# PhilippKath/concentus

Measured on NVIDIA B200. Metric: CELT decode audio-sec per sec (x realtime), 48k stereo, higher is better.
Workload: dtype int32

## Files before the change

concentus_b200/csrc/celt_bands.cuh:

```cuda
#pragma once
#include "celt_pvq.cuh"
#include "celt_rate.cuh"

namespace cb {

struct BandCtx {
    EcDec ec;
    int16_t *tmp;
    int i;
    int intensity, spread, tf_change;
    int remaining_bits;
    unsigned seed;
    bool dry;
};

struct SplitCtx {
    int inv, imid, iside, delta, itheta, qalloc;
};


CB_DEV_NOINLINE void haar1(int16_t *X, int N0, int stride) {
    N0 >>= 1;
    CB_NOUNROLL for (int i = 0; i < stride; i++)
        CB_NOUNROLL for (int j = 0; j < N0; j++) {
            int a = stride * 2 * j + i, b = stride * (2 * j + 1) + i;
            int t1 = mul16_16(23170, X[a]);
            int t2 = mul16_16(23170, X[b]);
            X[a] = (int16_t)pshr32(wadd(t1, t2), 15);
            X[b] = (int16_t)pshr32(wsub(t1, t2), 15);
        }
}

CB_DEV_NOINLINE void deinterleave_hadamard(int16_t *__restrict__ X, int16_t *__restrict__ tmp, int N0, int stride, int hadamard) {
    const int N = N0 * stride;
    const uint8_t *ordery = kOrdery + stride - 2;
    CB_NOUNROLL for (int i = 0; i < stride; i++) {
        const int row = hadamard ? ordery[i] : i;
        int16_t *d = tmp + row * N0;
        const int16_t *x = X + i;
        CB_NOUNROLL for (int j = 0; j < N0; j++) d[j] = x[j * stride];
    }
    CB_NOUNROLL for (int p = 0; p < N; p++) X[p] = tmp[p];
}
CB_DEV_NOINLINE void interleave_hadamard(int16_t *__restrict__ X, int16_t *__restrict__ tmp, int N0, int stride, int hadamard) {
    const int N = N0 * stride;
    const uint8_t *ordery = kOrdery + stride - 2;
    CB_NOUNROLL for (int i = 0; i < stride; i++) {
        const int row = hadamard ? ordery[i] : i;
        int16_t *d = tmp + i;
        const int16_t *x = X + row * N0;
        CB_NOUNROLL for (int j = 0; j < N0; j++) d[j * stride] = x[j];
    }
    CB_NOUNROLL for (int p = 0; p < N; p++) X[p] = tmp[p];
}

CB_DEV_NOINLINE void stereo_merge(int16_t *__restrict__ X, int16_t *__restrict__ Y, int mid, int N) {
    int xp = 0, side = 0;
    CB_NOUNROLL for (int j = 0; j < N; j++) {
        xp = mac16_16(xp, Y[j], X[j]);
        side = mac16_16(side, Y[j], Y[j]);
    }
    xp = mul16_32_q15(mid, xp);
    int mid2 = s16(mid >> 1);
    int El = wsub(wadd(mul16_16(mid2, mid2), side), wmul(2, xp));
    int Er = wadd(wadd(mul16_16(mid2, mid2), side), wmul(2, xp));
    if (Er < 161061 || El < 161061) {
        CB_NOUNROLL for (int j = 0; j < N; j++) Y[j] = X[j];
        return;
    }
    int kl = celt_ilog2(El) >> 1;
    int kr = celt_ilog2(Er) >> 1;
    int t = vshr32(El, (kl - 7) << 1);
    int lgain = celt_rsqrt_norm(t);
    t = vshr32(Er, (kr - 7) << 1);
    int rgain = celt_rsqrt_norm(t);
    if (kl < 7) kl = 7;
    if (kr < 7) kr = 7;
    CB_NOUNROLL for (int j = 0; j < N; j++) {
        int l = s16(mul16_16_p15(mid, X[j]));
        int r = Y[j];
        X[j] = (int16_t)pshr32(mul16_16(lgain, s16(l - r)), kl + 1);
        Y[j] = (int16_t)pshr32(mul16_16(rgain, s16(l + r)), kr + 1);
    }
}

CB_DEV int compute_qn(int N, int b, int offset, int pulse_cap, int stereo) {
    int N2 = 2 * N - 1;
    if (stereo && N == 2) N2--;
    int qb = sudiv(b + N2 * offset, N2);
    qb = imin(b - pulse_cap - (4 << kBitRes), qb);
    qb = imin(8 << kBitRes, qb);
    int qn;
    if (qb < (1 << kBitRes >> 1)) {
        qn = 1;
    } else {
        qn = kExp2Table8[qb & 0x7] >> (14 - (qb >> kBitRes));
        qn = (qn + 1) >> 1 << 1;
    }
    return qn;
}

CB_DEV void compute_theta(BandCtx &ctx, SplitCtx &sctx, int N, int *b, int B, int B0, int LM, int stereo, int *fill) {
    EcDec &ec = ctx.ec;
    int itheta = 0, inv = 0;
    int pulse_cap = kLogN[ctx.i] + LM * (1 << kBitRes);
    int offset = (pulse_cap >> 1) - (stereo && N == 2 ? kQThetaOffsetTwoPhase : kQThetaOffset);
    int qn = compute_qn(N, *b, offset, pulse_cap, stereo);
    if (stereo && ctx.i >= ctx.intensity) qn = 1;
    int tell = (int)ec.tell_frac();
    if (qn != 1) {
        if (stereo && N > 2) {
            const int p0 = 3;
            int x0 = qn / 2;
            unsigned ft = (unsigned)(p0 * (x0 + 1) + x0);
            int fs = (int)ec.decode(ft);
            int x;
            if (fs < (x0 + 1) * p0) x = fs / p0;
            else x = x0 + 1 + (fs - (x0 + 1) * p0);
            ec.update((unsigned)(x <= x0 ? p0 * x : (x - 1 - x0) + (x0 + 1) * p0),
                      (unsigned)(x <= x0 ? p0 * (x + 1) : (x - x0) + (x0 + 1) * p0), ft);
            itheta = x;
        } else if (B0 > 1 || stereo) {
            itheta = (int)ec.uint_((unsigned)qn + 1);
        } else {
            int fs = 1, fl = 0;
            int ft = ((qn >> 1) + 1) * ((qn >> 1) + 1);
            int fm = (int)ec.decode((unsigned)ft);
            if (fm < ((qn >> 1) * ((qn >> 1) + 1) >> 1)) {
                itheta = (int)((isqrt32(8 * (unsigned)fm + 1) - 1) >> 1);
                fs = itheta + 1;
                fl = itheta * (itheta + 1) >> 1;
            } else {
                itheta = (int)((2 * (unsigned)(qn + 1) - isqrt32(8 * (unsigned)(ft - fm - 1) + 1)) >> 1);
                fs = qn + 1 - itheta;
                fl = ft - ((qn + 1 - itheta) * (qn + 2 - itheta) >> 1);
            }
// ... 118 lines not shown
    int16_t *Y, *lowband2;
    int B0, mbits, sbits, itheta, rebalance0, gmid, gside, mid_first;
    int stage;
};

CB_DEV void quant_partition(BandCtx &ctx, LeafRec *leaves, int &nleaves, int16_t *X, int N, int b, int B, int16_t *lowband, int LM, int gain,
                            int fill) {
    PartFrame st[5];
    int sp = 0;
    st[0].X = X; st[0].lowband = lowband; st[0].N = N; st[0].b = b; st[0].B = B; st[0].LM = LM; st[0].gain = gain;
    st[0].fill = fill; st[0].shift = 0; st[0].stage = 0;
    while (sp >= 0) {
        PartFrame &f = st[sp];
        if (f.stage == 0) {
            const uint8_t *cache = pulse_cache(ctx.i, f.LM);
            if (f.LM != -1 && f.b > cache[cache[0]] + 12 && f.N > 2) {
                SplitCtx s;
                const int n = f.N >> 1;
                const int lm = f.LM - 1;
                int fl = f.fill;
                int bb = f.b;
                const int B0 = f.B;
                if (B0 == 1) fl = (fl & 1) | (fl << 1);
                const int Bn = (B0 + 1) >> 1;
                compute_theta(ctx, s, n, &bb, Bn, B0, lm, 0, &fl);
                int delta = s.delta;
                const int itheta = s.itheta;
                if (B0 > 1 && (itheta & 0x3fff)) {
                    if (itheta > 8192) delta -= delta >> (4 - lm);
                    else delta = imin(0, delta + (n << kBitRes >> (5 - lm)));
                }
                const int mbits = imax(0, imin(bb, (bb - delta) / 2));
                const int sbits = bb - mbits;
                ctx.remaining_bits -= s.qalloc;
                f.Y = f.X + n;
                f.lowband2 = f.lowband ? f.lowband + n : nullptr;
                f.B0 = B0; f.mbits = mbits; f.sbits = sbits; f.itheta = itheta;
                f.rebalance0 = ctx.remaining_bits;
                f.gmid = s16(mul16_16_p15(f.gain, s.imid));
                f.gside = s16(mul16_16_p15(f.gain, s.iside));
                f.N = n; f.LM = lm; f.B = Bn; f.fill = fl;
                f.stage = 1;
                f.mid_first = mbits >= sbits;
                PartFrame &c = st[sp + 1];
                c.N = n; c.B = Bn; c.LM = lm; c.stage = 0;
                if (f.mid_first) { c.X = f.X; c.lowband = f.lowband; c.b = mbits; c.gain = f.gmid; c.fill = fl; c.shift = f.shift; }
                else { c.X = f.Y; c.lowband = f.lowband2; c.b = sbits; c.gain = f.gside; c.fill = fl >> Bn; c.shift = f.shift + (B0 >> 1); }
                sp++;
            } else {
                partition_leaf(ctx, leaves, nleaves, f.X, f.N, f.b, f.B, f.lowband, f.LM, f.gain, f.fill, f.shift);
                sp--;
            }
        } else if (f.stage == 1) {
            PartFrame &c = st[sp + 1];
            c.N = f.N; c.B = f.B; c.LM = f.LM; c.stage = 0;
            if (f.mid_first) {
                int rebalance = f.mbits - (f.rebalance0 - ctx.remaining_bits);
                if (rebalance > 3 << kBitRes && f.itheta != 0) f.sbits += rebalance - (3 << kBitRes);
                c.X = f.Y; c.lowband = f.lowband2; c.b = f.sbits; c.gain = f.gside; c.fill = f.fill >> f.B; c.shift = f.shift + (f.B0 >> 1);
            } else {
                int rebalance = f.sbits - (f.rebalance0 - ctx.remaining_bits);
                if (rebalance > 3 << kBitRes && f.itheta != 16384) f.mbits += rebalance - (3 << kBitRes);
                c.X = f.X; c.lowband = f.lowband; c.b = f.mbits; c.gain = f.gmid; c.fill = f.fill; c.shift = f.shift;
            }
            f.stage = 2;
            sp++;
        } else {
            sp--;
        }
    }
}

CB_DEV unsigned quant_band(BandCtx &ctx, int16_t *X, int N, int b, int B, int16_t *lowband, int LM, int16_t *lowband_out, int gain,
                           int16_t *lowband_scratch, int fill) {
    int N0 = N, N_B = N, N_B0, B0 = B;
    int time_divide = 0, recombine = 0;
    int tf_change = ctx.tf_change;
    const int longBlocks = B0 == 1;
    unsigned cm = 0;
    N_B = (int)udiv((unsigned)N_B, (unsigned)B);
    if (N == 1) return quant_band_n1(ctx, X, nullptr, lowband_out);
    if (tf_change > 0) recombine = tf_change;
    if (ctx.dry) lowband = nullptr;
    if (lowband_scratch && lowband && (recombine || ((N_B & 1) == 0 && tf_change < 0) || B0 > 1)) {
        {
            int16_t *__restrict__ d = lowband_scratch;
            const int16_t *__restrict__ src = lowband;
            CB_NOUNROLL for (int j = 0; j < N; j++) d[j] = src[j];
        }
        lowband = lowband_scratch;
    }
    CB_NOUNROLL for (int k = 0; k < recombine; k++) {
        if (lowband) haar1(lowband, N >> k, 1 << k);
        fill = kBitInterleave[fill & 0xF] | kBitInterleave[fill >> 4] << 2;
    }
    B >>= recombine;
    N_B <<= recombine;
    while ((N_B & 1) == 0 && tf_change < 0) {
        if (lowband) haar1(lowband, N_B, B);
        fill |= fill << B;
        B <<= 1;
        N_B >>= 1;
        time_divide++;
        tf_change++;
    }
    B0 = B;
    N_B0 = N_B;
    if (B0 > 1 && lowband) deinterleave_hadamard(lowband, ctx.tmp, N_B >> recombine, B0 << recombine, longBlocks);

    LeafRec leaves[kMaxLeaves];
    int nleaves = 0;
    quant_partition(ctx, leaves, nleaves, X, N, b, B, lowband, LM, gain, fill);
    if (ctx.dry) return 0;
    {
        unsigned sd = ctx.seed;
        CB_NOUNROLL for (int l = 0; l < nleaves; l++) cm |= run_leaf(leaves[l], ctx.spread, sd);
        ctx.seed = sd;
    }

    if (B0 > 1) interleave_hadamard(X, ctx.tmp, N_B >> recombine, B0 << recombine, longBlocks);
    N_B = N_B0;
    B = B0;
    CB_NOUNROLL for (int k = 0; k < time_divide; k++) {
        B >>= 1;
        N_B <<= 1;
        cm |= cm >> B;
        haar1(X, N_B, B);
    }
    CB_NOUNROLL for (int k = 0; k < recombine; k++) {
        cm = kBitDeinterleave[cm];
        haar1(X, N0 >> k, 1 << k);
    }
    B <<= recombine;
    if (lowband_out) {
        const int n = s16(celt_sqrt(shl32(N0, 22)));
        int16_t *__restrict__ d = lowband_out;
        const int16_t *__restrict__ src = X;
        CB_NOUNROLL for (int j = 0; j < N0; j++) d[j] = (int16_t)mul16_16_q15(n, src[j]);
    }
    cm &= (1u << B) - 1;
    return cm;
}

CB_DEV void store_band(int16_t *g, const int16_t *x, int N, int LM) {
    if (LM == 3) {
        CB_NOUNROLL for (int j = 0; j < N; j += 8) *reinterpret_cast<int4 *>(g + j) = *reinterpret_cast<const int4 *>(x + j);
    } else if (LM == 2) {
        CB_NOUNROLL for (int j = 0; j < N; j += 4) *reinterpret_cast<int2 *>(g + j) = *reinterpret_cast<const int2 *>(x + j);
    } else if (LM == 1) {
        CB_NOUNROLL for (int j = 0; j < N; j += 2) *reinterpret_cast<int *>(g + j) = *reinterpret_cast<const int *>(x + j);
    } else {
        CB_NOUNROLL for (int j = 0; j < N; j++) g[j] = x[j];
    }
}

CB_DEV void quant_all_bands_dec(int start, int end, int16_t *X_, int16_t *Y_, uint8_t *collapse_masks, const int *pulses,
                                int shortBlocks, int spread, int dual_stereo, int intensity, const int *tf_res, int total_bits,
                                int balance, EcDec &ec_io, int LM, int codedBands, unsigned *seed, int16_t *norm, int16_t *tmp,
                                int16_t *xw, int16_t *lbs, bool dry) {
    const int M = 1 << LM;
    const int B = shortBlocks ? M : 1;
    const int C = Y_ != nullptr ? 2 : 1;
    const int norm_offset = M * kEBands[start];
    int16_t *norm2 = norm + M * kEBands[kNbEBands - 1] - norm_offset;
    int16_t *lowband_scratch = lbs;
    int lowband_offset = 0;
    int update_lowband = 1;
    BandCtx ctx;
    ctx.ec = ec_io;
    ctx.tmp = tmp;
    ctx.intensity = intensity; ctx.spread = spread; ctx.seed = *seed;
    ctx.dry = dry;
    CB_NOUNROLL for (int i = start; i < end; i++) {
        ctx.i = i;
        const int last = (i == end - 1);
        int16_t *X = xw;
        int16_t *Y = Y_ != nullptr ? xw + 176 : nullptr;
        const int N = M * kEBands[i + 1] - M * kEBands[i];
        const int tell = (int)ctx.ec.tell_frac();
        if (i != start) balance -= tell;
        const int remaining_bits = total_bits - tell - 1;
        ctx.remaining_bits = remaining_bits;
        int b;
        if (i <= codedBands - 1) {
            int curr_balance = sudiv(balance, imin(3, codedBands - i));
            b = imax(0, imin(16383, imin(remaining_bits + 1, pulses[i] + curr_balance)));
        } else {
            b = 0;
        }
        if (M * kEBands[i] - N >= M * kEBands[start] && (update_lowband || lowband_offset == 0)) lowband_offset = i;
        const int tf_change = tf_res[i];
        ctx.tf_change = tf_change;
        if (i == end - 1) lowband_scratch = nullptr;

        int effective_lowband = -1;
        unsigned x_cm, y_cm;
        if (lowband_offset != 0 && (spread != kSpreadAggressive || B > 1 || tf_change < 0)) {
            effective_lowband = imax(0, M * kEBands[lowband_offset] - norm_offset - N);
            int fold_start = lowband_offset;
            while (M * kEBands[--fold_start] > effective_lowband + norm_offset) {}
            int fold_end = lowband_offset - 1;
            while (M * kEBands[++fold_end] < effective_lowband + norm_offset + N) {}
            x_cm = y_cm = 0;
            int fold_i = fold_start;
            do {
                x_cm |= collapse_masks[fold_i * C + 0];
                y_cm |= collapse_masks[fold_i * C + C - 1];
            } while (++fold_i < fold_end);
        } else {
            x_cm = y_cm = (1u << B) - 1;
        }
        if (dual_stereo && i == intensity) {
            dual_stereo = 0;
            const int n = dry ? 0 : M * kEBands[i] - norm_offset;
            CB_NOUNROLL for (int j = 0; j < n; j++) norm[j] = (int16_t)((norm[j] + norm2[j]) >> 1);
        }
        int16_t *lb = effective_lowband != -1 ? norm + effective_lowband : nullptr;
        int16_t *lb_out = last ? nullptr : norm + M * kEBands[i] - norm_offset;

        enum { kMono, kDual, kStereo, kStereoN2 };
        int mode, npass;
        SplitCtx s;
        int mbits = 0, sbits = 0, rebalance0 = 0, sfill = 0, orig_fill = 0, sign = 1;
        int16_t *x2 = nullptr, *y2 = nullptr;
        if (Y != nullptr && !dual_stereo && N == 1) {
            x_cm = quant_band_n1(ctx, X, Y, lb_out);
            y_cm = x_cm;
            npass = 0;
            mode = kMono;
        } else if (dual_stereo) {
            mode = kDual; npass = 2;
        } else if (Y != nullptr) {
            orig_fill = sfill = (int)(x_cm | y_cm);
            int bs = b;
            compute_theta(ctx, s, N, &bs, B, B, LM, 1, &sfill);
            if (N == 2) {
                mode = kStereoN2; npass = 1;
                mbits = bs; sbits = 0;
                if (s.itheta != 0 && s.itheta != 16384) sbits = 1 << kBitRes;
                mbits -= sbits;
                const int c = s.itheta > 8192;
                ctx.remaining_bits -= s.qalloc + sbits;
                x2 = c ? Y : X;
                y2 = c ? X : Y;
                int sg = 0;
                if (sbits) sg = (int)ctx.ec.bits(1);
                sign = 1 - 2 * sg;
            } else {
                mode = kStereo; npass = 2;
                mbits = imax(0, imin(bs, (bs - s.delta) / 2));
                sbits = bs - mbits;
                ctx.remaining_bits -= s.qalloc;
                rebalance0 = ctx.remaining_bits;
// ... 125 lines not shown
```

concentus_b200/csrc/celt_pvq.cuh:

```cuda
#pragma once
#include "celt_ec.cuh"
#include "celt_tables.cuh"

namespace cb {

CB_DEV unsigned pvq_u(int n, int k) {
    int lo = n < k ? n : k, hi = n < k ? k : n;
    return kPvqU[kPvqURow[lo] + hi];
}
CB_DEV unsigned pvq_v(int n, int k) { return pvq_u(n, k) + pvq_u(n, k + 1); }
CB_DEV unsigned pvq_row(int r, int c) { return kPvqU[kPvqURow[r] + c]; }

CB_DEV_NOINLINE int pvq_decode_index(int n, int k, unsigned i, int16_t *y) {
    unsigned p;
    int s, k0, val;
    int yy = 0;
    while (n > 2) {
        unsigned q;
        if (k >= n) {
            const int rown = kPvqURow[n];
            p = kPvqU[rown + k + 1];
            s = -(int)(i >= p);
            i -= p & (unsigned)s;
            k0 = k;
            q = kPvqU[rown + n];
            if (q > i) {
                k = n;
                do p = pvq_row(--k, n);
                while (p > i);
            } else {
                CB_NOUNROLL for (p = kPvqU[rown + k]; p > i; p = kPvqU[rown + k]) k--;
            }
            i -= p;
            val = s16((k0 - k + s) ^ s);
            *y++ = (int16_t)val;
            yy = mac16_16(yy, val, val);
        } else {
            p = pvq_row(k, n);
            q = pvq_row(k + 1, n);
            if (p <= i && i < q) {
                i -= p;
                *y++ = 0;
            } else {
                s = -(int)(i >= q);
                i -= q & (unsigned)s;
                k0 = k;
                do p = pvq_row(--k, n);
                while (p > i);
                i -= p;
                val = s16((k0 - k + s) ^ s);
                *y++ = (int16_t)val;
                yy = mac16_16(yy, val, val);
            }
        }
        n--;
    }
    p = 2 * (unsigned)k + 1;
    s = -(int)(i >= p);
    i -= p & (unsigned)s;
    k0 = k;
    k = (int)((i + 1) >> 1);
    if (k) i -= 2 * (unsigned)k - 1;
    val = s16((k0 - k + s) ^ s);
    *y++ = (int16_t)val;
    yy = mac16_16(yy, val, val);
    s = -(int)i;
    val = s16((k + s) ^ s);
    *y = (int16_t)val;
    yy = mac16_16(yy, val, val);
    return yy;
}

CB_DEV_NOINLINE void exp_rotation1(int16_t *X, int len, int stride, int c, int s) {
    int ms = s16(-s);
    CB_NOUNROLL for (int i = 0; i < len - stride; i++) {
        int x1 = X[i], x2 = X[i + stride];
        X[i + stride] = (int16_t)pshr32(mac16_16(mul16_16(c, x2), s, x1), 15);
        X[i] = (int16_t)pshr32(mac16_16(mul16_16(c, x1), ms, x2), 15);
    }
    CB_NOUNROLL for (int i = len - 2 * stride - 1; i >= 0; i--) {
        int x1 = X[i], x2 = X[i + stride];
        X[i + stride] = (int16_t)pshr32(mac16_16(mul16_16(c, x2), s, x1), 15);
        X[i] = (int16_t)pshr32(mac16_16(mul16_16(c, x1), ms, x2), 15);
    }
}

CB_DEV void exp_rotation_dec(int16_t *X, int len, int stride, int K, int spread) {
    if (2 * K >= len || spread == kSpreadNone) return;
    int factor = spread == 1 ? 15 : spread == 2 ? 10 : 5;
    int gain = s16(celt_div(mul16_16(32767, len), len + factor * K));
    int theta = mul16_16_q15(gain, gain) >> 1;
    int c = celt_cos_norm(theta);
    int s = celt_cos_norm(s16(32767 - theta));
    int stride2 = 0;
    if (len >= 8 * stride) {
        stride2 = 1;
        while ((stride2 * stride2 + stride2) * stride + (stride >> 2) < len) stride2++;
    }
    len = (int)udiv((unsigned)len, (unsigned)stride);
    CB_NOUNROLL for (int i = 0; i < stride; i++) {
        int16_t *x = X + i * len;
        if (stride2) exp_rotation1(x, len, stride2, s, c);
        exp_rotation1(x, len, 1, c, s);
    }
}

CB_DEV void unit_gain(int E, int gain, int &g, int &k) {
    k = celt_ilog2(E) >> 1;
    int t = vshr32(E, 2 * (k - 7));
    g = s16(mul16_16_p15(celt_rsqrt_norm(t), gain));
}

CB_DEV unsigned alg_unquant_idx(int16_t *X, int N, int K, int spread, int B, unsigned idx, int gain) {
    int Ryy = pvq_decode_index(N, K, idx, X);
// ... 37 lines not shown
```

concentus_b200/csrc/celt_rate.cuh:

```cuda
#pragma once
#include "celt_ec.cuh"
#include "celt_tables.cuh"

namespace cb {

CB_DEV int band_width(int j) { return kEBands[j + 1] - kEBands[j]; }

CB_DEV int get_pulses(int i) { return i < 8 ? i : (8 + (i & 7)) << ((i >> 3) - 1); }

CB_DEV const uint8_t *pulse_cache(int band, int LM) { return kCacheBits + kCacheIndex[(LM + 1) * kNbEBands + band]; }

CB_MATH int bits2pulses(int band, int LM, int bits) {
    const uint8_t *cache = pulse_cache(band, LM);
    int lo = 0, hi = cache[0];
    bits--;
    CB_NOUNROLL for (int i = 0; i < kLogMaxPseudo; i++) {
        int mid = (lo + hi + 1) >> 1;
        if ((int)cache[mid] >= bits) hi = mid;
        else lo = mid;
    }
    if (bits - (lo == 0 ? -1 : (int)cache[lo]) <= (int)cache[hi] - bits) return lo;
    return hi;
}
CB_DEV int pulses2bits(int band, int LM, int pulses) {
    return pulses == 0 ? 0 : pulse_cache(band, LM)[pulses] + 1;
}

CB_DEV void init_caps(int *cap, int LM, int C) {
    CB_NOUNROLL for (int i = 0; i < kNbEBands; i++) {
        int N = band_width(i) << LM;
        cap[i] = (kCacheCaps[kNbEBands * (2 * LM + C - 1) + i] + 64) * C * N >> 2;
    }
}

struct AllocDecIo {
    EcDec &ec;
    CB_MEM int skip_flag(int , int , int , int ) { return ec.bit_logp(1); }
    CB_MEM int intensity(int , int start, int codedBands) { return start + (int)ec.uint_((unsigned)(codedBands + 1 - start)); }
    CB_MEM int dual_stereo(int ) { return ec.bit_logp(1); }
};

struct AllocScratch {
    int bits1[kNbEBands], bits2[kNbEBands], thresh[kNbEBands], trim_offset[kNbEBands];
};

template <class Io>
CB_DEV int compute_allocation(Io io, AllocScratch &sc, int start, int end, const int *offsets, const int *cap, int alloc_trim,
                              int *intensity, int *dual_stereo, int total, int *balance_out, int *pulses, int *ebits,
                              int *fine_priority, int C, int LM) {
    const int len = kNbEBands;
    int *bits1 = sc.bits1, *bits2 = sc.bits2, *thresh = sc.thresh, *trim_offset = sc.trim_offset;
    total = imax(total, 0);
    int skip_start = start;
    int skip_rsv = total >= 1 << kBitRes ? 1 << kBitRes : 0;
    total -= skip_rsv;
    int intensity_rsv = 0, dual_stereo_rsv = 0;
    if (C == 2) {
        intensity_rsv = kLog2Frac[end - start];
        if (intensity_rsv > total) intensity_rsv = 0;
        else {
            total -= intensity_rsv;
            dual_stereo_rsv = total >= 1 << kBitRes ? 1 << kBitRes : 0;
            total -= dual_stereo_rsv;
        }
    }
    CB_NOUNROLL for (int j = start; j < end; j++) {
        int w = band_width(j);
        thresh[j] = imax(C << kBitRes, (3 * w << LM << kBitRes) >> 4);
        trim_offset[j] = C * w * (alloc_trim - 5 - LM) * (end - j - 1) * (1 << (LM + kBitRes)) >> 6;
        if (w << LM == 1) trim_offset[j] -= C << kBitRes;
    }
    int lo = 1, hi = kNbAllocVectors - 1;
    do {
        int done = 0, psum = 0;
        int mid = (lo + hi) >> 1;
        CB_NOUNROLL for (int j = end; j-- > start;) {
            int bitsj = C * band_width(j) * kAllocVectors[mid * len + j] << LM >> 2;
            if (bitsj > 0) bitsj = imax(0, bitsj + trim_offset[j]);
            bitsj += offsets[j];
            if (bitsj >= thresh[j] || done) {
                done = 1;
                psum += imin(bitsj, cap[j]);
            } else if (bitsj >= C << kBitRes) {
                psum += C << kBitRes;
            }
        }
        if (psum > total) hi = mid - 1;
        else lo = mid + 1;
    } while (lo <= hi);
    hi = lo--;
    CB_NOUNROLL for (int j = start; j < end; j++) {
        int w = band_width(j);
        int b1 = C * w * kAllocVectors[lo * len + j] << LM >> 2;
// ... 147 lines not shown
```

concentus_b200/csrc/celt_tables.cuh:

```cuda
#pragma once
#include "celt_simt.cuh"

namespace cb {

#include "celt_tables_data.inc"

enum {
    kNbEBands = 21,
    kOverlap = 120,
    kShortMdct = 120,
    kMaxLM = 3,
    kMaxFrame = 960,
    kDecBuf = 2048,
    kCombMinPeriod = 15,
    kCombMaxPeriod = 1024,
    kBitRes = 3,
    kMaxFineBits = 8,
    kFineOffset = 21,
    kQThetaOffset = 4,
    kQThetaOffsetTwoPhase = 16,
    kLogMaxPseudo = 6,
    kAllocSteps = 6,
    kNbAllocVectors = 11,
    kLpcOrder = 24,
    kPreemphCoef0 = 27853,
};
enum { kSpreadNone = 0, kSpreadLight = 1, kSpreadNormal = 2, kSpreadAggressive = 3 };

CB_TABLE int8_t kEMeans[25] = {103, 100, 92, 85, 81, 77, 72, 70, 78, 75, 73, 71, 78, 74, 69, 72, 70, 74, 76, 71, 60, 60, 60, 60, 60};
CB_TABLE int16_t kPredCoef[4] = {29440, 26112, 21248, 16384};
CB_TABLE int16_t kBetaCoef[4] = {30147, 22282, 12124, 6554};
enum { kBetaIntra = 4915 };
CB_TABLE uint8_t kEProbModel[4][2][42] = {
    {{72, 127, 65, 129, 66, 128, 65, 128, 64, 128, 62, 128, 64, 128, 64, 128, 92, 78, 92, 79, 92, 78, 90, 79, 116, 41, 115, 40, 114, 40, 132, 26, 132, 26, 145, 17, 161, 12, 176, 10, 177, 11},
     {24, 179, 48, 138, 54, 135, 54, 132, 53, 134, 56, 133, 55, 132, 55, 132, 61, 114, 70, 96, 74, 88, 75, 88, 87, 74, 89, 66, 91, 67, 100, 59, 108, 50, 120, 40, 122, 37, 97, 43, 78, 50}},
    {{83, 78, 84, 81, 88, 75, 86, 74, 87, 71, 90, 73, 93, 74, 93, 74, 109, 40, 114, 36, 117, 34, 117, 34, 143, 17, 145, 18, 146, 19, 162, 12, 165, 10, 178, 7, 189, 6, 190, 8, 177, 9},
     {23, 178, 54, 115, 63, 102, 66, 98, 69, 99, 74, 89, 71, 91, 73, 91, 78, 89, 86, 80, 92, 66, 93, 64, 102, 59, 103, 60, 104, 60, 117, 52, 123, 44, 138, 35, 133, 31, 97, 38, 77, 45}},
    {{61, 90, 93, 60, 105, 42, 107, 41, 110, 45, 116, 38, 113, 38, 112, 38, 124, 26, 132, 27, 136, 19, 140, 20, 155, 14, 159, 16, 158, 18, 170, 13, 177, 10, 187, 8, 192, 6, 175, 9, 159, 10},
     {21, 178, 59, 110, 71, 86, 75, 85, 84, 83, 91, 66, 88, 73, 87, 72, 92, 75, 98, 72, 105, 58, 107, 54, 115, 52, 114, 55, 112, 56, 129, 51, 132, 40, 150, 33, 140, 29, 98, 35, 77, 42}},
    {{42, 121, 96, 66, 108, 43, 111, 40, 117, 44, 123, 32, 120, 36, 119, 33, 127, 33, 134, 34, 139, 21, 147, 23, 152, 20, 158, 25, 154, 26, 166, 21, 173, 16, 184, 13, 184, 10, 150, 13, 139, 15},
     {22, 178, 63, 114, 74, 82, 84, 83, 92, 82, 103, 62, 96, 72, 96, 67, 101, 73, 107, 72, 113, 55, 118, 52, 125, 52, 118, 52, 117, 55, 135, 49, 137, 39, 157, 32, 145, 29, 97, 33, 77, 40}},
};
CB_TABLE uint8_t kSmallEnergyIcdf[3] = {2, 1, 0};
CB_TABLE uint8_t kTrimIcdf[11] = {126, 124, 119, 109, 87, 41, 19, 9, 4, 2, 0};
CB_TABLE uint8_t kSpreadIcdf[4] = {25, 23, 2, 0};
CB_TABLE uint8_t kTapsetIcdf[3] = {2, 1, 0};
CB_TABLE int8_t kTfSelect[4][8] = {
    {0, -1, 0, -1, 0, -1, 0, -1}, {0, -1, 0, -2, 1, 0, 1, -1}, {0, -2, 0, -3, 2, 0, 1, -1}, {0, -2, 0, -3, 3, 0, 1, -1}};
CB_TABLE uint8_t kLog2Frac[24] = {0, 8, 13, 16, 19, 21, 23, 24, 26, 27, 28, 29, 30, 31, 32, 32, 33, 34, 34, 35, 36, 36, 37, 37};
CB_TABLE int16_t kCombGains[3][3] = {{10048, 7112, 4248}, {15200, 8784, 0}, {26208, 3280, 0}};
CB_TABLE uint8_t kOrdery[30] = {1, 0, 3, 0, 2, 1, 7, 0, 4, 3, 6, 1, 5, 2, 15, 0, 8, 7, 12, 3, 11, 4, 14, 1, 9, 6, 13, 2, 10, 5};
CB_TABLE uint8_t kBitInterleave[16] = {0, 1, 1, 1, 2, 3, 3, 3, 2, 3, 3, 3, 2, 3, 3, 3};
CB_TABLE uint8_t kBitDeinterleave[16] = {0x00, 0x03, 0x0C, 0x0F, 0x30, 0x33, 0x3C, 0x3F, 0xC0, 0xC3, 0xCC, 0xCF, 0xF0, 0xF3, 0xFC, 0xFF};
CB_TABLE int16_t kExp2Table8[8] = {16384, 17866, 19483, 21247, 23170, 25267, 27554, 30048};

struct FftPlan {
    int16_t nfft;
    int8_t scale_shift;
    int8_t tw_shift;
    int8_t nstages;
    int8_t radix[5];
    int16_t m[5];
};
CB_TABLE FftPlan kFftPlan[4] = {
    {480, 8, 0, 5, {4, 2, 4, 3, 5}, {1, 4, 8, 32, 96}},
    {240, 7, 1, 4, {4, 4, 3, 5, 0}, {1, 4, 16, 48, 0}},
    {120, 6, 2, 4, {4, 2, 3, 5, 0}, {1, 4, 8, 24, 0}},
    {60, 5, 3, 3, {4, 3, 5, 0, 0}, {1, 4, 12, 0, 0}},
};
enum { kFftScale = 17476 };

enum {
    OPUS_OK_ = 0, OPUS_BAD_ARG_ = -1, OPUS_BUFFER_TOO_SMALL_ = -2, OPUS_INTERNAL_ERROR_ = -3,
    OPUS_INVALID_PACKET_ = -4, OPUS_UNIMPLEMENTED_ = -5, OPUS_INVALID_STATE_ = -6, OPUS_ALLOC_FAIL_ = -7,
};
enum { kBwNarrow = 1101, kBwMedium = 1102, kBwWide = 1103, kBwSuperWide = 1104, kBwFull = 1105 };

CB_TABLE uint8_t kBinToBand[100] = {
    0, 1, 2, 3, 4, 5, 6, 7, 8, 8, 9, 9, 10, 10, 11, 11, 12, 12, 12, 12, 13, 13, 13, 13, 14, 14, 14, 14,
    15, 15, 15, 15, 15, 15, 16, 16, 16, 16, 16, 16, 17, 17, 17, 17, 17, 17, 17, 17,
    18, 18, 18, 18, 18, 18, 18, 18, 18, 18, 18, 18,
    19, 19, 19, 19, 19, 19, 19, 19, 19, 19, 19, 19, 19, 19, 19, 19, 19, 19,
    20, 20, 20, 20, 20, 20, 20, 20, 20, 20, 20, 20, 20, 20, 20, 20, 20, 20, 20, 20, 20, 20};

CB_TABLE int16_t kIntensityThresholds[21] = {1, 2, 3, 4, 5, 6, 7, 8, 16, 24, 36, 44, 50, 56, 62, 67, 72, 79, 88, 106, 134};
CB_TABLE int16_t kIntensityHisteresis[21] = {1, 1, 1, 1, 1, 1, 1, 2, 2, 2, 2, 2, 2, 2, 3, 3, 4, 5, 6, 8, 8};

CB_DEV const int16_t *fft_bitrev(int s) {
    return s == 0 ? kFftBitrev480 : s == 1 ? kFftBitrev240 : s == 2 ? kFftBitrev120 : kFftBitrev60;
}

}
```

concentus_b200/csrc/opus_capi.cu:

```cuda
#define CB_SMALL_CODE 1
#include <cuda_runtime.h>

#include <cstdarg>
#include <cstdio>
#include <cstdlib>
#include <cstring>
#include <mutex>
#include <unordered_set>
#include <vector>

#include "../../include/opus_b200.h"
#include "host_runtime.h"
#include "opus_decoder_dev.cuh"
#include "opus_multistream.h"

using namespace cb;

struct OpusDecoder {
    uint32_t magic;
    int32_t slot;
    uint64_t gen;
    int32_t host_current;
    int32_t device;
    CbDecState st;
};
static const uint32_t kDecMagic = 0x0B200DECu;

#ifndef CB_PARSE_THREADS
#define CB_PARSE_THREADS 128
#endif
#ifndef CB_PARSE_MINBLOCKS
#define CB_PARSE_MINBLOCKS 8
#endif
#ifndef CB_WPB
#define CB_WPB 4
#endif
#ifndef CB_SYNTH_MINBLOCKS
#define CB_SYNTH_MINBLOCKS 8
#endif

struct IrView {
    CbPacketIR *pk;
    CbFrameIR *fr;
    int16_t *X;
    int *sig;
    CbSigRange *range;
    int kmax;
    int xstride;
    int sigstride;
    int Fc;
};

__global__ void __launch_bounds__(CB_PARSE_THREADS, CB_PARSE_MINBLOCKS)
parse_kernel(const CbCallCtx *call_ctx, const uint8_t *data, const int64_t *offs, const int32_t *lens, int n, int F,
             int f0, int f1, int call_f0, int R, int cap, int decode_fec, IrView ir) {
    const int runs = (f1 - f0 + R - 1) / R;
    const int t = blockIdx.x * blockDim.x + threadIdx.x;
    if (t >= n * runs) return;
    const int s = t / runs, r = t - s * runs;
    ParseScratch ps;
    const int first = f0 + r * R;
    const int last = first + R < f1 ? first + R : f1;
    opus_parse_run(call_ctx[s], data, offs + (size_t)s * F, lens + (size_t)s * F, call_f0, first, last, cap, decode_fec, ir.kmax, ir.xstride,
                   ir.pk + (size_t)s * ir.Fc, ir.fr + (size_t)s * ir.Fc * ir.kmax, ir.X + (size_t)s * ir.Fc * ir.xstride, f0, ps);
}

__global__ void call_ctx_kernel(const CbDecState *pool, const int *slots, CbCallCtx *out, int n) {
    const int s = blockIdx.x * blockDim.x + threadIdx.x;
    if (s < n) call_ctx_from_state(out[s], pool + slots[s]);
}

__global__ void __launch_bounds__(CB_WPB * 32, CB_SYNTH_MINBLOCKS)
synth_kernel(CbDecState *pool, const int *slots, IrView ir, int16_t *pcm, int n, int F, int f0, int f1, int pcm_F, int pcm_f0,
             int cap, int row, int *rets, PlcScratch *plc) {
    extern __shared__ __align__(16) unsigned char smem[];
    const int warp = threadIdx.x >> 5, lane = threadIdx.x & 31;
    const int s = blockIdx.x * CB_WPB + warp;
    if (s >= n) return;
    SynthScratch &S = *(reinterpret_cast<SynthScratch *>(smem) + warp);
    CbDecState *st = pool + slots[s];
    WarpTeam tm{lane};
    for (int f = f0; f < f1; f++) {
        const size_t slot = (size_t)s * ir.Fc + (f - f0);
        int16_t *out = pcm + ((size_t)s * pcm_F + f - pcm_f0) * row;
        int r = opus_synth_packet(tm, st, S, plc[s], ir.pk[slot], ir.fr + slot * ir.kmax, ir.X + slot * ir.xstride, out, cap,
                                  ir.sig + slot * ir.sigstride, ir.range + slot);
        if (lane == 0) rets[(size_t)s * F + f] = r;
        __syncwarp();
    }
}

__device__ __forceinline__ int deemph_pair_stereo(const int *x, int n, int16_t *pcm_lr, int c, int m, int gain, unsigned pairmask) {
    for (int j = 0; j < n; j += 8) {
        const int4 a = *reinterpret_cast<const int4 *>(x + j);
        const int4 b = *reinterpret_cast<const int4 *>(x + j + 4);
        const int xs[8] = {a.x, a.y, a.z, a.w, b.x, b.y, b.z, b.w};
        unsigned w[4];
#pragma unroll
        for (int u = 0; u < 8; u++) {
            int t = wadd(xs[u], m);
            m = mul16_32_q15(kPreemphCoef0, t);
            int v = sig2word16(t);
            if (gain >= 0) { int g = mul16_32_p16(v, gain); v = g > 32767 ? 32767 : (g < -32767 ? -32767 : g); }
            if (u & 1) w[u >> 1] |= (unsigned)(v & 0xffff) << 16;
            else w[u >> 1] = (unsigned)(v & 0xffff);
        }
        const unsigned o0 = __shfl_xor_sync(pairmask, c == 0 ? w[2] : w[0], 1);
        const unsigned o1 = __shfl_xor_sync(pairmask, c == 0 ? w[3] : w[1], 1);
        const unsigned l0 = c == 0 ? w[0] : o0, l1 = c == 0 ? w[1] : o1;
        const unsigned r0 = c == 0 ? o0 : w[2], r1 = c == 0 ? o1 : w[3];
        uint4 out;
        out.x = __byte_perm(l0, r0, 0x5410);
        out.y = __byte_perm(l0, r0, 0x7632);
        out.z = __byte_perm(l1, r1, 0x5410);
        out.w = __byte_perm(l1, r1, 0x7632);
        *reinterpret_cast<uint4 *>(pcm_lr + (j + (c == 0 ? 0 : 4)) * 2) = out;
    }
    return m;
}

__global__ void __launch_bounds__(128)
deemph_kernel(CbDecState *pool, const int *slots, IrView ir, int16_t *pcm, int n, int f0, int f1, int pcm_F, int pcm_f0, int cap, int row) {
    const int t = blockIdx.x * blockDim.x + threadIdx.x;
    const int s = t >> 1, c = t & 1;
    if (s >= n) return;
    CbDecState *st = pool + slots[s];
    const int channels = st->channels;
    if (c >= channels) return;
    const int ds = st->downsample;
    const int gain = st->decode_gain ? celt_exp2(s16(mul16_16_p15(21771, st->decode_gain))) : -1;
    const unsigned pairmask = 3u << ((threadIdx.x & 31) & ~1);
    const bool paired = channels == 2 && ds == 1;
    int m = st->preemph_memD[c];
    for (int f = f0; f < f1; f++) {
        const size_t slot = (size_t)s * ir.Fc + (f - f0);
        int16_t *out = pcm + ((size_t)s * pcm_F + (f - pcm_f0)) * row;
        const CbSigRange rg = ir.range[slot];
        if (rg.end <= rg.begin) continue;
// ... 106 lines not shown
    DevBuf d_blob, d_eoffs, d_elens, d_erets, d_mserr, d_map, d_epcm[2], d_extent;
    cudaEvent_t ev_gather[2] = {nullptr, nullptr};
    size_t ir_budget = (size_t)16 << 30;
    size_t ir_budget_host = (size_t)6 << 30;
    int run_len = 3;
    int parse_wave_blocks = 0;
    int max_waves = 1;
    PinBuf h_stage, h_slots, h_misc;
    long long launches = 0;
    float last_ms = 0.f;
    struct Timed { cudaEvent_t a, b; int stage; };
    std::vector<Timed> timed;
    std::vector<cudaEvent_t> ev_pool;
    double stage_ms[5] = {0, 0, 0, 0, 0};
    long long stage_launches[5] = {0, 0, 0, 0, 0};
    int smem_per_block = 0;
    std::mutex deferred_mu;
    std::vector<std::pair<int, const void *>> deferred;
};
Ctx g_ctxs[kCbMaxDevices];
thread_local int tl_device = -1;
int g_default_device = -1;
inline int cur_device() {
    const int d = tl_device >= 0 ? tl_device : g_default_device;
    return d < 0 || d >= kCbMaxDevices ? 0 : d;
}
#define g (g_ctxs[cur_device()])

enum { kStageStates = 4096 };

void release_slot_locked(OpusDecoder *d);
bool ctx_init_locked() {
    if (g.tried) {
        if (g.ok) {
            cudaSetDevice(g.device);
            if (!g.deferred.empty()) {
                std::lock_guard<std::mutex> lk(g.deferred_mu);
                for (auto &pr : g.deferred)
                    if (pr.first >= 0 && pr.first < g.pool_cap && g.reg[pr.first].owner == pr.second) {
                        g.reg[pr.first].owner = nullptr;
                        g.reg[pr.first].gen++;
                        g.free_slots.push_back(pr.first);
                    }
                g.deferred.clear();
            }
        }
        return g.ok;
    }
    g.tried = true;
    g.device = cur_device();
    int ndev = 0;
    if (cudaGetDeviceCount(&ndev) != cudaSuccess || ndev <= 0) {
        fprintf(stderr, "concentus_b200: no CUDA device available — this library has no CPU path\n");
        return false;
    }
    if (g.device >= ndev) return false;
    if (cudaSetDevice(g.device) != cudaSuccess) return false;
    int prio_lo = 0, prio_hi = 0;
    cudaDeviceGetStreamPriorityRange(&prio_lo, &prio_hi);
    if (!getenv("CB200_PRIO")) prio_hi = prio_lo;
    if (cudaStreamCreateWithPriority(&g.stream, cudaStreamNonBlocking, prio_hi) != cudaSuccess) return false;
    if (cudaStreamCreateWithPriority(&g.copy_stream, cudaStreamNonBlocking, prio_hi) != cudaSuccess) return false;
    if (cudaStreamCreateWithPriority(&g.parse_stream, cudaStreamNonBlocking, prio_lo) != cudaSuccess) return false;
    if (cudaStreamCreateWithPriority(&g.synth_stream, cudaStreamNonBlocking, prio_hi) != cudaSuccess) return false;
    cudaEventCreate(&g.ev0);
    cudaEventCreate(&g.ev1);
    for (int i = 0; i < 2; i++) {
        cudaEventCreateWithFlags(&g.ev_chunk[i], cudaEventDisableTiming);
        cudaEventCreateWithFlags(&g.ev_copy[i], cudaEventDisableTiming);
        cudaEventCreateWithFlags(&g.ev_parse[i], cudaEventDisableTiming);
        cudaEventCreateWithFlags(&g.ev_synth[i], cudaEventDisableTiming);
        cudaEventCreateWithFlags(&g.ev_deemph[i], cudaEventDisableTiming);
        cudaEventCreateWithFlags(&g.ev_gather[i], cudaEventDisableTiming);
    }
    cudaEventCreateWithFlags(&g.ev_call, cudaEventDisableTiming);
    if (const char *e = getenv("CB200_IR_MB")) g.ir_budget = (size_t)atol(e) << 20;
    if (const char *e = getenv("CB200_IR_HOST_MB")) g.ir_budget_host = (size_t)atol(e) << 20;
    if (const char *e = getenv("CB200_RUN")) g.run_len = atoi(e) > 0 ? atoi(e) : 5;
    if (const char *e = getenv("CB200_WAVES")) g.max_waves = atoi(e);
    {
        int per_sm = 0, dev = 0, sms = 0;
        cudaGetDevice(&dev);
        cudaDeviceGetAttribute(&sms, cudaDevAttrMultiProcessorCount, dev);
        if (cudaOccupancyMaxActiveBlocksPerMultiprocessor(&per_sm, parse_kernel, CB_PARSE_THREADS, 0) == cudaSuccess)
            g.parse_wave_blocks = per_sm * sms;
        if (getenv("CB200_NO_WAVE_SIZING")) g.parse_wave_blocks = 0;
    }
    {
        size_t free_b = 0, total_b = 0;
        if (cudaMemGetInfo(&free_b, &total_b) == cudaSuccess && g.ir_budget > free_b / 10) g.ir_budget = free_b / 10;
    }
    g.smem_per_block = (int)(CB_WPB * sizeof(SynthScratch));
    cudaFuncSetAttribute(synth_kernel, cudaFuncAttributeMaxDynamicSharedMemorySize, g.smem_per_block);
    cudaFuncSetAttribute(parse_kernel, cudaFuncAttributePreferredSharedMemoryCarveout, 0);
    if (!g.h_stage.reserve(sizeof(CbDecState) * 64)) return false;
    if (!g.d_stage.reserve(sizeof(CbDecState) * 64)) return false;
    g.ok = (cudaGetLastError() == cudaSuccess);
    return g.ok;
}

bool pool_reserve_locked(int need_total) {
    if (need_total <= g.pool_cap) return true;
    int ncap = g.pool_cap ? g.pool_cap : 64;
    while (ncap < need_total) ncap *= 2;
    CbDecState *np = nullptr;
    if (cudaMalloc(&np, sizeof(CbDecState) * (size_t)ncap) != cudaSuccess) return false;
    if (g.pool) {
        cudaMemcpyAsync(np, g.pool, sizeof(CbDecState) * (size_t)g.pool_cap, cudaMemcpyDeviceToDevice, g.stream);
        cudaStreamSynchronize(g.stream);
        cudaFree(g.pool);
    }
    for (int i = ncap - 1; i >= g.pool_cap; i--) g.free_slots.push_back(i);
    g.reg.resize(ncap, SlotInfo{nullptr, 0});
    g.pool = np;
    g.pool_cap = ncap;
    return true;
}

inline bool resident(const OpusDecoder *d) {
    return d->device == g.device && d->slot >= 0 && d->slot < g.pool_cap && g.reg[d->slot].owner == d && g.reg[d->slot].gen == d->gen;
}
void release_elsewhere(OpusDecoder *d) {
    if (d->slot >= 0 && d->device >= 0 && d->device < kCbMaxDevices && d->device != g.device) {
        Ctx &o = g_ctxs[d->device];
        std::lock_guard<std::mutex> lk(o.deferred_mu);
        o.deferred.emplace_back(d->slot, (const void *)d);
        d->slot = -1;
    }
}

int make_host_current_locked(OpusDecoder *d) {
    if (d->host_current) return OPUS_OK;
    if (d->device != g.device || d->slot < 0 || d->slot >= g.pool_cap || g.reg[d->slot].gen != d->gen) return OPUS_INVALID_STATE;
    if (cudaMemcpyAsync(&d->st, g.pool + d->slot, sizeof(CbDecState), cudaMemcpyDeviceToHost, g.stream) != cudaSuccess)
        return OPUS_INTERNAL_ERROR;
    if (cudaStreamSynchronize(g.stream) != cudaSuccess) return OPUS_INTERNAL_ERROR;
    d->host_current = 1;
    return OPUS_OK;
}

void release_slot_locked(OpusDecoder *d) {
    release_elsewhere(d);
    if (d->slot >= 0 && d->slot < g.pool_cap && g.reg[d->slot].owner == d) {
        g.reg[d->slot].owner = nullptr;
        g.reg[d->slot].gen++;
        g.free_slots.push_back(d->slot);
    }
    d->slot = -1;
}

int make_resident_locked(OpusDecoder **st, int n, int *h_slots) {
    int need_new = 0;
    for (int i = 0; i < n; i++) {
        OpusDecoder *d = st[i];
        if (!d || d->magic != kDecMagic) return OPUS_BAD_ARG;
        if (!resident(d)) need_new++;
    }
    if (n > 1) {
        std::unordered_set<const void *> seen;
        seen.reserve((size_t)n * 2);
        for (int i = 0; i < n; i++)
            if (!seen.insert(st[i]).second) return OPUS_BAD_ARG;
    }
    int in_use = g.pool_cap - (int)g.free_slots.size();
    if (!pool_reserve_locked(in_use + need_new)) return OPUS_ALLOC_FAIL;
    std::vector<int> up_idx;
    for (int i = 0; i < n; i++) {
        OpusDecoder *d = st[i];
        if (resident(d)) {
            if (d->host_current) up_idx.push_back(i);
        } else {
            if (!d->host_current) {
                int rc = make_host_current_locked(d);
                if (rc != OPUS_OK) return rc;
            }
            release_elsewhere(d);
            d->slot = g.free_slots.back();
// ... 882 lines not shown
```

Measured before the change: 174,400.

## Stage PVQ and pulse-cache tables in shared memory; drop hadamard copy-back

The parse kernel now copies the PVQ U table, its row index, and the pulse-cache tables into block shared memory at launch. PVQ decoding and bits-to-pulses lookups then read from shared memory instead of constant or global tables. The shared-memory carveout is sized from the kernel's static footprint so the minimum blocks per SM still fit. Separately, deinterleave/interleave_hadamard write into separate buffers (tmp and an xh buffer reusing lowband scratch) instead of copying back in place, which also removes the lowband copy when only B0>1. The cost is a per-block table-load prologue with a __syncthreads and extra shared memory that may reduce L1 or occupancy. Aliasing lbs as both xh and lowband_scratch is a correctness risk.

```diff
diff --git a/concentus_b200/csrc/celt_bands.cuh b/concentus_b200/csrc/celt_bands.cuh
--- a/concentus_b200/csrc/celt_bands.cuh
+++ b/concentus_b200/csrc/celt_bands.cuh
@@ -7,6 +7,7 @@
 struct BandCtx {
     EcDec ec;
     int16_t *tmp;
+    int16_t *xh;
     int i;
     int intensity, spread, tf_change;
     int remaining_bits;
@@ -31,27 +32,23 @@
         }
 }
 
-CB_DEV_NOINLINE void deinterleave_hadamard(int16_t *__restrict__ X, int16_t *__restrict__ tmp, int N0, int stride, int hadamard) {
-    const int N = N0 * stride;
+CB_DEV_NOINLINE void deinterleave_hadamard(const int16_t *__restrict__ X, int16_t *__restrict__ d0, int N0, int stride, int hadamard) {
     const uint8_t *ordery = kOrdery + stride - 2;
     CB_NOUNROLL for (int i = 0; i < stride; i++) {
         const int row = hadamard ? ordery[i] : i;
-        int16_t *d = tmp + row * N0;
+        int16_t *d = d0 + row * N0;
         const int16_t *x = X + i;
         CB_NOUNROLL for (int j = 0; j < N0; j++) d[j] = x[j * stride];
     }
-    CB_NOUNROLL for (int p = 0; p < N; p++) X[p] = tmp[p];
-}
-CB_DEV_NOINLINE void interleave_hadamard(int16_t *__restrict__ X, int16_t *__restrict__ tmp, int N0, int stride, int hadamard) {
-    const int N = N0 * stride;
+}
+CB_DEV_NOINLINE void interleave_hadamard(const int16_t *__restrict__ X, int16_t *__restrict__ d0, int N0, int stride, int hadamard) {
     const uint8_t *ordery = kOrdery + stride - 2;
     CB_NOUNROLL for (int i = 0; i < stride; i++) {
         const int row = hadamard ? ordery[i] : i;
-        int16_t *d = tmp + i;
+        int16_t *d = d0 + i;
         const int16_t *x = X + row * N0;
         CB_NOUNROLL for (int j = 0; j < N0; j++) d[j * stride] = x[j];
     }
-    CB_NOUNROLL for (int p = 0; p < N; p++) X[p] = tmp[p];
 }
 
 CB_DEV_NOINLINE void stereo_merge(int16_t *__restrict__ X, int16_t *__restrict__ Y, int mid, int N) {
@@ -336,7 +333,7 @@
     if (N == 1) return quant_band_n1(ctx, X, nullptr, lowband_out);
     if (tf_change > 0) recombine = tf_change;
     if (ctx.dry) lowband = nullptr;
-    if (lowband_scratch && lowband && (recombine || ((N_B & 1) == 0 && tf_change < 0) || B0 > 1)) {
+    if (lowband_scratch && lowband && (recombine || ((N_B & 1) == 0 && tf_change < 0))) {
         {
             int16_t *__restrict__ d = lowband_scratch;
             const int16_t *__restrict__ src = lowband;
@@ -360,11 +357,14 @@
     }
     B0 = B;
     N_B0 = N_B;
-    if (B0 > 1 && lowband) deinterleave_hadamard(lowband, ctx.tmp, N_B >> recombine, B0 << recombine, longBlocks);
+    if (B0 > 1 && lowband) {
+        deinterleave_hadamard(lowband, ctx.tmp, N_B >> recombine, B0 << recombine, longBlocks);
+        lowband = ctx.tmp;
+    }
 
     LeafRec leaves[kMaxLeaves];
     int nleaves = 0;
-    quant_partition(ctx, leaves, nleaves, X, N, b, B, lowband, LM, gain, fill);
+    quant_partition(ctx, leaves, nleaves, B0 > 1 ? ctx.xh : X, N, b, B, lowband, LM, gain, fill);
     if (ctx.dry) return 0;
     {
         unsigned sd = ctx.seed;
@@ -372,7 +372,7 @@
         ctx.seed = sd;
     }
 
-    if (B0 > 1) interleave_hadamard(X, ctx.tmp, N_B >> recombine, B0 << recombine, longBlocks);
+    if (B0 > 1) interleave_hadamard(ctx.xh, X, N_B >> recombine, B0 << recombine, longBlocks);
     N_B = N_B0;
     B = B0;
     CB_NOUNROLL for (int k = 0; k < time_divide; k++) {
@@ -423,6 +423,7 @@
     BandCtx ctx;
     ctx.ec = ec_io;
     ctx.tmp = tmp;
+    ctx.xh = lbs;
     ctx.intensity = intensity; ctx.spread = spread; ctx.seed = *seed;
     ctx.dry = dry;
     CB_NOUNROLL for (int i = start; i < end; i++) {
diff --git a/concentus_b200/csrc/celt_pvq.cuh b/concentus_b200/csrc/celt_pvq.cuh
--- a/concentus_b200/csrc/celt_pvq.cuh
+++ b/concentus_b200/csrc/celt_pvq.cuh
@@ -6,10 +6,10 @@
 
 CB_DEV unsigned pvq_u(int n, int k) {
     int lo = n < k ? n : k, hi = n < k ? k : n;
-    return kPvqU[kPvqURow[lo] + hi];
+    return CB_TAB_PVQ_U[CB_TAB_PVQ_UROW[lo] + hi];
 }
 CB_DEV unsigned pvq_v(int n, int k) { return pvq_u(n, k) + pvq_u(n, k + 1); }
-CB_DEV unsigned pvq_row(int r, int c) { return kPvqU[kPvqURow[r] + c]; }
+CB_DEV unsigned pvq_row(int r, int c) { return CB_TAB_PVQ_U[CB_TAB_PVQ_UROW[r] + c]; }
 
 CB_DEV_NOINLINE int pvq_decode_index(int n, int k, unsigned i, int16_t *y) {
     unsigned p;
@@ -18,18 +18,18 @@
     while (n > 2) {
         unsigned q;
         if (k >= n) {
-            const int rown = kPvqURow[n];
-            p = kPvqU[rown + k + 1];
+            const int rown = CB_TAB_PVQ_UROW[n];
+            p = CB_TAB_PVQ_U[rown + k + 1];
             s = -(int)(i >= p);
             i -= p & (unsigned)s;
             k0 = k;
-            q = kPvqU[rown + n];
+            q = CB_TAB_PVQ_U[rown + n];
             if (q > i) {
                 k = n;
                 do p = pvq_row(--k, n);
                 while (p > i);
             } else {
-                CB_NOUNROLL for (p = kPvqU[rown + k]; p > i; p = kPvqU[rown + k]) k--;
+                CB_NOUNROLL for (p = CB_TAB_PVQ_U[rown + k]; p > i; p = CB_TAB_PVQ_U[rown + k]) k--;
             }
             i -= p;
             val = s16((k0 - k + s) ^ s);
diff --git a/concentus_b200/csrc/celt_rate.cuh b/concentus_b200/csrc/celt_rate.cuh
--- a/concentus_b200/csrc/celt_rate.cuh
+++ b/concentus_b200/csrc/celt_rate.cuh
@@ -8,7 +8,7 @@
 
 CB_DEV int get_pulses(int i) { return i < 8 ? i : (8 + (i & 7)) << ((i >> 3) - 1); }
 
-CB_DEV const uint8_t *pulse_cache(int band, int LM) { return kCacheBits + kCacheIndex[(LM + 1) * kNbEBands + band]; }
+CB_DEV const uint8_t *pulse_cache(int band, int LM) { return CB_TAB_CACHE_BITS + CB_TAB_CACHE_INDEX[(LM + 1) * kNbEBands + band]; }
 
 CB_MATH int bits2pulses(int band, int LM, int bits) {
     const uint8_t *cache = pulse_cache(band, LM);
diff --git a/concentus_b200/csrc/celt_tables.cuh b/concentus_b200/csrc/celt_tables.cuh
--- a/concentus_b200/csrc/celt_tables.cuh
+++ b/concentus_b200/csrc/celt_tables.cuh
@@ -26,6 +26,32 @@
     kPreemphCoef0 = 27853,
 };
 enum { kSpreadNone = 0, kSpreadLight = 1, kSpreadNormal = 2, kSpreadAggressive = 3 };
+
+#if defined(__CUDACC__) && defined(CB_STAGE_A_SMEM_TABLES)
+struct StageATables {
+    uint32_t pvq_u[sizeof(kPvqU) / sizeof(kPvqU[0])];
+    int16_t pvq_urow[sizeof(kPvqURow) / sizeof(kPvqURow[0])];
+    int16_t cache_index[sizeof(kCacheIndex) / sizeof(kCacheIndex[0])];
+    uint8_t cache_bits[sizeof(kCacheBits)];
+};
+static __shared__ StageATables sStageA;
+#define CB_TAB_PVQ_U sStageA.pvq_u
+#define CB_TAB_PVQ_UROW sStageA.pvq_urow
+#define CB_TAB_CACHE_INDEX sStageA.cache_index
+#define CB_TAB_CACHE_BITS sStageA.cache_bits
+static __device__ __forceinline__ void stage_a_tables_load() {
+    for (int j = threadIdx.x; j < (int)(sizeof(kPvqU) / sizeof(kPvqU[0])); j += blockDim.x) sStageA.pvq_u[j] = kPvqU[j];
+    for (int j = threadIdx.x; j < (int)(sizeof(kPvqURow) / sizeof(kPvqURow[0])); j += blockDim.x) sStageA.pvq_urow[j] = kPvqURow[j];
+    for (int j = threadIdx.x; j < (int)(sizeof(kCacheIndex) / sizeof(kCacheIndex[0])); j += blockDim.x) sStageA.cache_index[j] = kCacheIndex[j];
+    for (int j = threadIdx.x; j < (int)sizeof(kCacheBits); j += blockDim.x) sStageA.cache_bits[j] = kCacheBits[j];
+    __syncthreads();
+}
+#else
+#define CB_TAB_PVQ_U kPvqU
+#define CB_TAB_PVQ_UROW kPvqURow
+#define CB_TAB_CACHE_INDEX kCacheIndex
+#define CB_TAB_CACHE_BITS kCacheBits
+#endif
 
 CB_TABLE int8_t kEMeans[25] = {103, 100, 92, 85, 81, 77, 72, 70, 78, 75, 73, 71, 78, 74, 69, 72, 70, 74, 76, 71, 60, 60, 60, 60, 60};
 CB_TABLE int16_t kPredCoef[4] = {29440, 26112, 21248, 16384};
diff --git a/concentus_b200/csrc/opus_capi.cu b/concentus_b200/csrc/opus_capi.cu
--- a/concentus_b200/csrc/opus_capi.cu
+++ b/concentus_b200/csrc/opus_capi.cu
@@ -1,4 +1,5 @@
 #define CB_SMALL_CODE 1
+#define CB_STAGE_A_SMEM_TABLES 1
 #include <cuda_runtime.h>
 
 #include <cstdarg>
@@ -54,6 +55,7 @@
 __global__ void __launch_bounds__(CB_PARSE_THREADS, CB_PARSE_MINBLOCKS)
 parse_kernel(const CbCallCtx *call_ctx, const uint8_t *data, const int64_t *offs, const int32_t *lens, int n, int F,
              int f0, int f1, int call_f0, int R, int cap, int decode_fec, IrView ir) {
+    cb::stage_a_tables_load();
     const int runs = (f1 - f0 + R - 1) / R;
     const int t = blockIdx.x * blockDim.x + threadIdx.x;
     if (t >= n * runs) return;
@@ -326,6 +328,17 @@
         int per_sm = 0, dev = 0, sms = 0;
         cudaGetDevice(&dev);
         cudaDeviceGetAttribute(&sms, cudaDevAttrMultiProcessorCount, dev);
+        int carveout = 0;
+        cudaFuncAttributes fa;
+        int smem_sm = 0, smem_rsv = 0;
+        if (cudaFuncGetAttributes(&fa, parse_kernel) == cudaSuccess && fa.sharedSizeBytes > 0 &&
+            cudaDeviceGetAttribute(&smem_sm, cudaDevAttrMaxSharedMemoryPerMultiprocessor, dev) == cudaSuccess && smem_sm > 0 &&
+            cudaDeviceGetAttribute(&smem_rsv, cudaDevAttrReservedSharedMemoryPerBlock, dev) == cudaSuccess) {
+            const size_t need = (size_t)CB_PARSE_MINBLOCKS * (fa.sharedSizeBytes + (size_t)smem_rsv);
+            carveout = (int)((need * 100 + (size_t)smem_sm - 1) / (size_t)smem_sm);
+            if (carveout > 100) carveout = 100;
+        }
+        cudaFuncSetAttribute(parse_kernel, cudaFuncAttributePreferredSharedMemoryCarveout, carveout);
         if (cudaOccupancyMaxActiveBlocksPerMultiprocessor(&per_sm, parse_kernel, CB_PARSE_THREADS, 0) == cudaSuccess)
             g.parse_wave_blocks = per_sm * sms;
         if (getenv("CB200_NO_WAVE_SIZING")) g.parse_wave_blocks = 0;
@@ -336,7 +349,6 @@
     }
     g.smem_per_block = (int)(CB_WPB * sizeof(SynthScratch));
     cudaFuncSetAttribute(synth_kernel, cudaFuncAttributeMaxDynamicSharedMemorySize, g.smem_per_block);
-    cudaFuncSetAttribute(parse_kernel, cudaFuncAttributePreferredSharedMemoryCarveout, 0);
     if (!g.h_stage.reserve(sizeof(CbDecState) * 64)) return false;
     if (!g.d_stage.reserve(sizeof(CbDecState) * 64)) return false;
     g.ok = (cudaGetLastError() == cudaSuccess);
```

After: 176,100 (median of 6 runs). About the same (+1.0%).
